# richardshuai/ExPecto

Hardware: AMD Instinct MI355X
Metric: variants/sec (200 windows × 2002 feats) at 1/2/4/8 MI355X; HBM GB/s vs peak (higher is better)
Workload: dtype fp32 in/out (f16x3: power-of-2-scaled 2-way fp16 split = 22-bit operands, 3 MFMA products, fp32 accumulate; bf16x6 recompute on fp16 overflow)

## Files before the change

### expecto_amd/csrc/beluga.hip

```cpp
#include <hip/hip_runtime.h>

#include <algorithm>
#include <array>
#include <cassert>
#include <cstdint>
#include <cstdlib>
#include <cstring>
#include <map>
#include <mutex>
#include <tuple>
#include <string>
#include <vector>

#include "common.h"
#include "gemm_kernel.h"
#include "seg_plan.h"

namespace expecto {

static_assert(kStrandFwd == EXPECTO_STRAND_FWD && kStrandRc == EXPECTO_STRAND_RC && kStrandBoth == EXPECTO_STRAND_BOTH &&
              EXPECTO_EINVAL == -1, "seg_plan.h restates the strand modes and the refusal code");
constexpr int kNFeat = 2002;
constexpr int kFc1In = 67840;
constexpr int kFc1Out = 2003;
// ... 1302 lines not shown
  float* h1 = nullptr;
  long long* a_rows = nullptr;
  long long* c_rows = nullptr;
  int fc2_rows = 0;
  int* win_seg_d = nullptr;
  int* alt_w_d = nullptr;
  int* copy_w_d = nullptr;
  int* seg_var_d = nullptr;
  int seg_var_cap = 0;
  int* win_off_d = nullptr;
  int* win_row_d = nullptr;
  int* fc_perm_d = nullptr;
  hipStream_t st2 = nullptr;
  hipEvent_t pev[16] = {};
  bool overlap = true;
  float* DA = nullptr;
  float* D0 = nullptr;
  float* D1 = nullptr;
  uint8_t* delta_codes = nullptr;
  int* seg_tab = nullptr;
  float* slab_mask = nullptr;
  int win_cap = 0;
  size_t bytes = 0;
  std::vector<void*> allocs;
  int precision = EXPECTO_PRECISION_BF16X6;
  int fc_splits = kFcSplitsDefault;
  int fc2_splits = kFc2SplitsDefault;
  double fc1_m_order_mb = 80.0;
  int fc1_order = 3;
  int fc1_m_group = 8;
  bool fc_wide = true;
  int conv_tile = 0;
  bool conv_ea = true;
  bool fc_skinny = true;
  int fc1_narrow = -1;
  int conv_narrow = -1;
  bool narrow_scope = false;
  int seg_chunk_windows = 0;
  bool seg_merge_strands = true;
  int cus = 0;
  bool pool_one_pass = true;
  bool pool_fused = true;
  float* seam = nullptr;
  float* edge = nullptr;
  size_t seam_cap = 0, edge_cap = 0;
  bool fuse_conv1 = true;
  bool kmer_on = true;
  float* kmer = nullptr;
  uint64_t kmer_key = 0;
  bool kmer_quad = true;
  int kmer_state = 1;
  bool fk_on = true;
  int fk_role = 4;
  float* fkw = nullptr;
  int* fk_sw = nullptr;
  float* fk_cs = nullptr;
  float* fk_seq[3] = {};
  long long fk_seq_rows = 0;
  long long* fk_grows = nullptr;
  long long* fk_wrows = nullptr;
  int* fk_prow = nullptr;
  unsigned* fk_mask = nullptr;
  int fk_slice = 24576;
  float* fk_part = nullptr;
  float* fk_h1 = nullptr;
  long long* fk_arows = nullptr;
// ... 246 lines not shown
    if (idx < 0) return;
    (void)hipEventRecord(h->ev_pool[idx + 1], st);
    h->pending_launch.push_back(rec);
  }
};

struct LayerTimer {
  expecto_beluga* h;
  int layer;
  int idx = -1;
  hipStream_t st;
  LayerTimer(expecto_beluga* hh, int l, hipStream_t s) : h(hh), layer(hh->timer_base + l), st(s) {
    if (!h->profiling) return;
    if (h->ev_next + 2 > h->ev_pool.size()) resolve_events(h);
    idx = (int)h->ev_next;
    h->ev_next += 2;
    (void)hipEventRecord(h->ev_pool[idx], st);
  }
  ~LayerTimer() {
    if (idx < 0) return;
    (void)hipEventRecord(h->ev_pool[idx + 1], st);
    h->pending.push_back({layer, idx});
  }
};

struct DeltaScope {
  expecto_beluga* h;
  explicit DeltaScope(expecto_beluga* hh) : h(hh) { h->timer_base = kNumLayers; }
  ~DeltaScope() { h->timer_base = 0; }
};

thread_local int g_precision = EXPECTO_PRECISION_BF16X6;
thread_local bool g_conv_ea = true;

int act_fmt() {
  return g_precision == EXPECTO_PRECISION_BF16X6 ? 1 : g_precision == EXPECTO_PRECISION_F16X3 ? 2 : 0;
}
int act_bytes() { return act_fmt() == 1 ? 6 : 4; }
bool planes_gemm() { return g_precision != EXPECTO_PRECISION_FP32; }
long long gemm_bm() { return planes_gemm() ? X6P_BM : GBM; }
float exp2i(int e) { return std::ldexp(1.0f, e); }

int conv_tile_rows(const expecto_beluga* h, int l, bool pool, long long M, int n_tiles) {
  if (g_precision != EXPECTO_PRECISION_F16X3) return (int)gemm_bm();
  if (h->conv_tile) return h->conv_tile;
  const int cus = h->cus > 0 ? h->cus : 256;
  auto cost = [&](int bm, double per_row) {
    const long long blocks = (M + bm - 1) / bm * n_tiles;
    return (double)((blocks + cus - 1) / cus) * bm * per_row;
  };
  return cost(384, 1.0) * 1.1 <= cost(256, 1.0) ? 384 : 256;
}

int conv_narrow_cols(int l) { return l == 1 || l == 2 ? 128 : 64; }
bool conv_narrow(const expecto_beluga* h, int l, long long M, int bm, int n_tiles) {
  if (g_precision != EXPECTO_PRECISION_F16X3 || l < 1 || l > 4) return false;
  if (h->conv_narrow >= 0) return h->conv_narrow != 0;
  if (!h->narrow_scope) return false;
  const long long cus = h->cus > 0 ? h->cus : 256;
  const int nc = conv_narrow_cols(l);
  const long long narrow = (M + 255) / 256 * ((kConv[l].cout + nc - 1) / nc), wide = (M + bm - 1) / bm * n_tiles;
  return narrow <= cus && wide < cus;
}

template <int LAYER, int EPI>
int launch_gemm(const GemmArgs& a, int splits, hipStream_t st, int bm = 0) {
// ... 21 lines not shown
          if (g_conv_ea)
            beluga_conv_h3p<LAYER, EPI, 256 | 64 | H3P_FUSE_CONV1, 4><<<dim3((unsigned)nblk), dim3(512), 0, st>>>(a);
          else
            beluga_conv_h3p<LAYER, EPI, 256 | H3P_FUSE_CONV1, 4><<<dim3((unsigned)nblk), dim3(512), 0, st>>>(a);
        } else {
          EXPECTO_REQUIRE(false, "fused conv1: conv2 + pool1 only");
        }
      } else if (a.n_tile_cols == 64) {
        if constexpr ((LAYER == 5 || LAYER == 6) && EPI == EPI_RELU) {
          EXPECTO_REQUIRE(bm == 256 && a.n_tiles * 64 >= a.n_store, "64-column conv tiles: 256 rows");
          beluga_conv_h3p_narrow<LAYER, EPI, 4><<<dim3((unsigned)nblk), dim3(512), 0, st>>>(a);
        } else {
          EXPECTO_REQUIRE(false, "64-column conv tiles: conv5 / conv6 only");
        }
      } else if (a.n_tile_cols == 128) {
        if constexpr (LAYER == 3 || LAYER == 4) {
          EXPECTO_REQUIRE(bm == 256 && a.n_tiles == 4 && a.n_store == 480, "128-column conv tiles: conv3 / conv4");
          beluga_conv_h3p_narrow<LAYER, EPI, 8><<<dim3((unsigned)nblk), dim3(512), 0, st>>>(a);
        } else {
          EXPECTO_REQUIRE(false, "128-column conv tiles: conv3 / conv4 only");
        }
      } else if (bm == 384)
        beluga_conv_h3r<LAYER, EPI><<<dim3((unsigned)nblk), dim3(256), 0, st>>>(a);
      else if (g_conv_ea)
        beluga_conv_h3p<LAYER, EPI, 256 | 64, 4><<<dim3((unsigned)nblk), dim3(512), 0, st>>>(a);
      else
        beluga_conv_h3p<LAYER, EPI, 256, 4><<<dim3((unsigned)nblk), dim3(512), 0, st>>>(a);
    } else if constexpr (EPI == EPI_PARTIAL) {
      EXPECTO_REQUIRE(a.n_tile_cols == 0 || a.n_tile_cols == FCW_BN || a.n_tile_cols == 112 ||
                          a.n_tile_cols == 16 * FCS_NB,
                      "FC tile width: 0 (160), 336, 112 or 32 columns");
      EXPECTO_REQUIRE((long long)a.n_tiles * (a.n_tile_cols ? a.n_tile_cols : GBN) >= a.n_store,
                      "FC N tiles do not cover the stored columns");
      if (a.n_tile_cols == FCW_BN)
        beluga_fc_h3w<LAYER, EPI><<<dim3((unsigned)nblk), dim3(512), 0, st>>>(a);
      else if (a.n_tile_cols == 112)
        beluga_fc_h3w_narrow<LAYER, EPI><<<dim3((unsigned)nblk), dim3(512), 0, st>>>(a);
      else if (a.n_tile_cols == 16 * FCS_NB) {
        EXPECTO_REQUIRE(a.m_tiles == 1 && a.M <= 32 && !a.ks_mask, "skinny FC tiles: one tile of <= 32 rows");
        beluga_fc_h3s<LAYER, EPI><<<dim3((unsigned)nblk), dim3(64 * 2 * FCS_NB), 0, st>>>(a);
      }
      else
        beluga_fc_h3p<LAYER, EPI><<<dim3((unsigned)nblk), dim3(512), 0, st>>>(a);
    } else {
      beluga_fc_h3p<LAYER, EPI><<<dim3((unsigned)nblk), dim3(512), 0, st>>>(a);
    }
  } else
    beluga_gemm<LAYER, EPI, kWM, kMinBlocks, GBK, kPipe><<<dim3((unsigned)nblk), dim3(64 * kWM), 0, st>>>(a);
  return check_launch("beluga_gemm");
}

int run_conv1(expecto_beluga* h, const float* x, const uint8_t* codes, long long code_stride, int n_src, int mode,
              long long row0, int nb, int len, int out_rows, hipStream_t st, float* dst = nullptr) {
  LayerTimer lt(h, 0, st);
  if (h->profiling) h->macs[h->timer_base + 0] += (double)nb * (len - 7) * 320 * 32;
  if (g_precision == EXPECTO_PRECISION_F16X3 && h->w1h) {
    dim3 grid((len - 7 + C1H_ROWS - 1) / C1H_ROWS, nb);
    beluga_conv1_h3<<<grid, dim3(320), 0, st>>>(x, codes, code_stride, n_src, mode, row0,
                                                reinterpret_cast<const _Float16*>(h->w1h), h->cs1, h->b1,
                                                dst ? dst : h->P, out_rows, len, exp2i(h->sx[0]), h->ovf);
    return check_launch("beluga_conv1_h3");
  }
  dim3 grid((len - 7 + C1_T - 1) / C1_T, nb);
  beluga_conv1<<<grid, dim3(320), 0, st>>>(x, codes, code_stride, n_src, mode, row0, h->w1, h->b1,
                                           dst ? dst : h->P, out_rows, len, act_fmt(), exp2i(h->sx[0]), h->ovf);
  return check_launch("beluga_conv1");
}

// ... 451 lines not shown
            g * kFkKb + s * kFkKb / kFkSlabs, kFkKb / kFkSlabs, pr.cnt[g], lay);
      else {
        row += lay;
        ++mslot;
      }
    }
  }
  add(x, w_rows, 100LL * 640, 9 * kFkKb, kFkTailK / GBK, n, n);
  EXPECTO_REQUIRE(G.n <= FCK_MAX && blk < (1LL << 31), "Karatsuba FC1 descriptors");
  EXPECTO_REQUIRE(row <= part_cap, "Karatsuba FC1 partial rows");
  {
    LayerTimer lt(h, 6, st);
    if (h->profiling) {
      if (!mask) {
        h->macs[h->timer_base + 6] += macs;
      } else {
        for (int i = 0; i < G.n; ++i) {
          const FcDesc& d = G.d[i];
          int rc = count_desc_macs(h, d.mask, d.m_tiles, (double)d.M / d.m_tiles * kFc1Out * d.nk * GBK, st);
          if (rc) return rc;
        }
      }
    }
    G.rr = mask ? 0 : 1;
    const long long mtt = blk / G.n_tiles;
    const bool narrow = !mask && fc1_narrow(h, mtt);
    if (narrow) {
      G.n_tiles = kHidLd / (16 * kFcNarrowNb);
      for (int i = 0; i < G.n; ++i) G.d[i].blk0 = G.d[i].blk0 / (kHidLd / FCW_BN) * G.n_tiles;
    }
    const long long grid = G.rr ? (mtt + 7) / 8 * 8 * G.n_tiles : mtt * G.n_tiles;
    if (narrow)
      beluga_fc_h3k_narrow<<<dim3((unsigned)grid), dim3(512), 0, st>>>(G);
    else
      beluga_fc_h3k<0><<<dim3((unsigned)grid), dim3(512), 0, st>>>(G);
    int rc = check_launch("beluga_fc_h3k");
    if (rc) return rc;
  }
  return prow ? fk_reduce(h, part, prow, n, h1, st) : EXPECTO_OK;
}

void fk_slice_tables(const std::vector<FkWin>& ws, int i0, int i1, int T6, std::vector<long long>& grows,
                     FkProducts& pr, std::vector<int>& prow, std::vector<int>* rgrp = nullptr,
                     std::vector<int>* ginfo = nullptr) {
  const int n = i1 - i0;
  std::vector<int> gi(n);
  std::vector<long long> gst;
  std::vector<unsigned> need;
  for (int i = i0; i < i1; ++i) {
    const FkWin& w = ws[i];
    if (i == i0 || !fk_same_group(w, ws[i - 1])) {
      gst.push_back(((long long)w.blk * T6 + fk_group_of(w.off6)) * 640);
      need.push_back(0u);
    }
    gi[i - i0] = (int)gst.size() - 1;
    for (int j = 0; j < 4; ++j) need.back() |= 1u << kFkRole[fk_role_of(w.off6)][j];
    if (ginfo && gi[i - i0] * 2 == (int)ginfo->size()) {
      ginfo->push_back(w.blk);
      ginfo->push_back(fk_group_of(w.off6));
    }
  }
  const int ng = (int)gst.size();
  std::vector<int> ridx((size_t)9 * ng, -1);
  grows.clear();
  if (rgrp) rgrp->clear();
  for (int g = 0; g < 9; ++g) {
    pr.off[g] = (int)grows.size();
    int c = 0;
// ... 36 lines not shown
  return run_fc2(h, h->h1, R, y, st, c_rows);
}

int count_slab_macs(expecto_beluga* h, const unsigned* mask, int tiles, long long nb, hipStream_t st) {
  if (!h->macs_d) {
    float* f = nullptr;
    int rc = dalloc(h, &f, 4 * kNumLayers);
    if (rc) return rc;
    h->macs_d = reinterpret_cast<double*>(f);
    EXPECTO_HIP_CHECK(hipMemsetAsync(h->macs_d, 0, 2 * kNumLayers * sizeof(double), st));
  }
  const double per_bit = (double)nb * kFc1Out * kFc1In / ((double)tiles * h->fc_splits);
  slab_macs<<<dim3(1), dim3(64), 0, st>>>(mask, tiles, per_bit, h->macs_d + kNumLayers + 6);
  return check_launch("slab_macs");
}

int count_desc_macs(expecto_beluga* h, const unsigned* mask, int tiles, double per_tile, hipStream_t st) {
  if (!h->macs_d) {
    float* f = nullptr;
    int rc = dalloc(h, &f, 4 * kNumLayers);
    if (rc) return rc;
    h->macs_d = reinterpret_cast<double*>(f);
    EXPECTO_HIP_CHECK(hipMemsetAsync(h->macs_d, 0, 2 * kNumLayers * sizeof(double), st));
  }
  slab_macs<<<dim3(1), dim3(64), 0, st>>>(mask, tiles, per_tile, h->macs_d + h->timer_base + 6);
  return check_launch("slab_macs");
}

int forward_chunk(expecto_beluga* h, const float* x, const uint8_t* codes, long long code_stride, int n_src,
                  int mode, long long row0, int nb, float* y, hipStream_t st) {
  int rc;
  g_precision = h->precision;
  g_conv_ea = h->conv_ea;
  struct Scope {
    expecto_beluga* h;
    ~Scope() { h->narrow_scope = false; }
  } scope{h};
  h->narrow_scope = true;
  const bool kmer = use_kmer(h, x);
  const bool fuse = !kmer && fuse_conv1(h, x);
  const C1Src f1{codes, code_stride, n_src, mode, row0, kLen};
  if (!kmer && !fuse && (rc = run_conv1(h, x, codes, code_stride, n_src, mode, row0, nb, kLen, kS1, st))) return rc;
  float* src = h->P;
  float* dst = h->Q;
  for (int l = 0; l < 5; ++l) {
    const ConvGeo& g = kConv[l];
    if (l == 0 && kmer)
      rc = run_conv2_kmer(h, f1, nb, g.t_valid, g.s_out, dst, st);
    else
      rc = run_conv(h, l, src, dst, nb, g.s_in, g.t_valid, g.s_out, g.pool != 0, st, l == 0 && fuse ? &f1 : nullptr);
    if (rc) return rc;
    std::swap(src, dst);
  }
  if (fk_use(h)) return fk_windows(h, src, nb, y, st, nullptr);
  return run_fc(h, src, nullptr, nb, y, st);
}

int ensure_delta(expecto_beluga* h) {
  if (h->DA) return EXPECTO_OK;
  const size_t pad = 16 * 640;
  const size_t da = (size_t)h->max_batch * kDA[6] * 640 + pad, dd = (size_t)h->max_batch * kDW[6] * 640 + pad;
  float *pc = nullptr, *tb = nullptr;
  int rc;
  if ((rc = dalloc(h, &h->DA, act_alloc(da))) || (rc = dalloc(h, &h->D0, act_alloc(dd))) ||
      (rc = dalloc(h, &h->D1, act_alloc(dd))) || (rc = dalloc(h, &pc, (size_t)h->max_batch * kC1PatStride / 4)) ||
      (rc = dalloc(h, &tb, (size_t)h->max_batch * kSegTab)) ||
// ... 351 lines not shown
    if (planes_gemm()) {
      const int tiles = (int)((na + gemm_bm() - 1) / gemm_bm());
      unsigned* md = reinterpret_cast<unsigned*>(h->slab_mask);
      EXPECTO_HIP_CHECK(hipMemsetAsync(md, 0, tiles * sizeof(unsigned), st));
      fc1_slab_mask_seg<<<dim3((na + 255) / 256), dim3(256), 0, st>>>(
          widx + f0, na, h->win_seg_d, h->win_off_d, ck.s0, pl.ss, pl.g.L, c.phi, h->seg_tab, (int)gemm_bm(),
          kFc1In / h->fc_splits, md);
      if ((rc = check_launch("fc1_slab_mask_seg"))) return rc;
      mask = md;
      if (h->profiling) {
        if ((rc = count_slab_macs(h, md, tiles, na, st))) return rc;
        frac = 0.0;
      }
    }
    DeltaScope ds(h);
    if (gather2) {
      float* h1a = h1_rows(h, h->fc2_rows);
      if ((rc = run_fc1(h, h->Q, h->a_rows, na, h1a, st, mask, frac, fn)) ||
          (rc = run_fc2(h, h1a, na, pr->y_alt, st, acrow)))
        return rc;
    } else if ((rc = run_fc(h, h->Q, h->a_rows, na, pr->y_alt, st, h->c_rows, mask, frac, fn))) {
      return rc;
    }
  }
  if ((rc = flush2())) return rc;
  return seg_copy_tail(c, ck);
}

int forward_segments(expecto_beluga* h, const uint8_t* codes, int n_seg, int L, long long code_stride, int mode,
                     const int* win_seg, const int* win_off, const int* win_row, int n_win, float* y,
                     hipStream_t st, const SegPairs* pr = nullptr) {
  g_precision = h->precision;
  g_conv_ea = h->conv_ea;
  SegPlan pl;
  const char* refusal = nullptr;
  if (seg_plan({n_seg, L, mode, win_seg, win_off, win_row, n_win, pr ? pr->var_pos : nullptr,
                pr ? pr->strand_stride : n_win, h->max_batch, p_floats(h->max_batch) - 16 * 640,
                q_floats(h->max_batch) - 16 * 640, h->seg_merge_strands, h->seg_chunk_windows, fk_use_seg(h), fk_cap(h)},
               pl, &refusal)) {
    set_error(refusal);
    return EXPECTO_EINVAL;
  }
  int rc;
  if (pr && (rc = ensure_delta(h))) return rc;
  if (n_win > h->win_cap) {
    for (int** b : {&h->win_seg_d, &h->win_off_d, &h->win_row_d, &h->alt_w_d, &h->copy_w_d, &h->fc_perm_d}) {
      if (*b) EXPECTO_HIP_CHECK(hipFree(*b));
      *b = nullptr;
    }
    h->win_cap = 0;
    for (int** b : {&h->win_seg_d, &h->win_off_d, &h->win_row_d}) EXPECTO_HIP_CHECK(hipMalloc(b, n_win * sizeof(int)));
    for (int** b : {&h->alt_w_d, &h->copy_w_d}) EXPECTO_HIP_CHECK(hipMalloc(b, 2 * n_win * sizeof(int)));
    EXPECTO_HIP_CHECK(hipMalloc(&h->fc_perm_d, 4 * n_win * sizeof(int)));
    h->win_cap = n_win;
  }
  if (pr && n_seg > h->seg_var_cap) {
    if (h->seg_var_d) EXPECTO_HIP_CHECK(hipFree(h->seg_var_d));
    h->seg_var_d = nullptr;
    h->seg_var_cap = 0;
    EXPECTO_HIP_CHECK(hipMalloc(&h->seg_var_d, n_seg * sizeof(int)));
    h->seg_var_cap = n_seg;
  }
  std::vector<HostCopy> copies;
  if (pr) {
    copies.push_back({h->seg_var_d, pr->var_pos, n_seg * sizeof(int)});
    copies.push_back({h->alt_w_d, pl.alt_w.data(), pl.alt_w.size() * sizeof(int)});
    copies.push_back({h->copy_w_d, pl.copy_w.data(), pl.copy_w.size() * sizeof(int)});
  }
  if (win_row) copies.push_back({h->win_row_d, win_row, n_win * sizeof(int)});
  copies.push_back({h->win_seg_d, win_seg, n_win * sizeof(int)});
  copies.push_back({h->win_off_d, win_off, n_win * sizeof(int)});
  if (!pl.fc_perm.empty()) copies.push_back({h->fc_perm_d, pl.fc_perm.data(), pl.fc_perm.size() * sizeof(int)});
  if ((rc = stage_copies(h, copies, st))) return rc;
  const SegGeo& g = pl.g;
  const SegCall c{h, pl, st, (pr && h->st2) ? h->st2 : st, pr, SegDims{L, g.T1, g.P1, g.T3, g.T4, g.S5, g.T5, g.T6},
                  make_int4(pl.ph[0], pl.ph[1], pl.ph[2], pl.ph[3]),
                  make_int4(pl.ph_idx[0], pl.ph_idx[1], pl.ph_idx[2], pl.ph_idx[3]), act_bytes(), codes, code_stride,
                  mode, y, win_row ? h->win_row_d : nullptr};
  for (size_t ci = 0; ci < pl.chunks.size(); ++ci) {
    const int s0 = pl.chunks[ci].first, s1 = pl.chunks[ci].second;
    const SegChunk ck{ci, s0, s1 - s0, pl.vfirst[s0], pl.vfirst[s1] - pl.vfirst[s0], (long long)(s1 - s0) * pl.n_ph};
    PQSwap pq{h, false};
    if ((rc = seg_trunk(c, ck, pq))) return rc;
    if (ck.nw > 0 && (rc = pl.fkm ? seg_fc_karatsuba(c, ck) : seg_fc_direct(c, ck))) return rc;
    if (pr && (rc = seg_st_wait(c, h->pev[13]))) return rc;
  }
  return EXPECTO_OK;
}
int forward_pairs(expecto_beluga* h, const uint8_t* ref, const uint8_t* alt, int n, long long stride,
                  const int* var_pos, int mode, float* y_ref, float* y_alt, long long strand_stride, hipStream_t st) {
  g_precision = h->precision;
  g_conv_ea = h->conv_ea;
  const int strands = mode == EXPECTO_STRAND_BOTH ? 2 : 1;
  int rc;
  if ((rc = ensure_delta(h))) return rc;
  const int eb = act_bytes();
  const int nv_max = std::max(1, h->max_batch / strands);
  hipStream_t sa = h->st2 ? h->st2 : st;
  for (int v0 = 0; v0 < n; v0 += nv_max) {
    const int nv = std::min(nv_max, n - v0), R = strands * nv;
    if ((rc = stream_order(st, sa, h->pev[0]))) return rc;
    const bool kmer = use_kmer(h, nullptr);
    const bool fuse = !kmer && fuse_conv1(h, nullptr);
    const C1Src f1{ref + (long long)v0 * stride, stride, nv, mode, 0, kLen};
    if (!kmer && !fuse && (rc = run_conv1(h, nullptr, f1.codes, stride, nv, mode, 0, R, kLen, kS1, st))) return rc;
    if (kmer || fuse) {
      delta_codes2<<<dim3((R + 4) / 5), dim3(5 * kC1PatStride), 0, sa>>>(alt, stride, nv, v0, var_pos, h->delta_codes, R);
      if ((rc = check_launch("delta_codes2"))) return rc;
      DeltaScope ds(h);
      if (fuse && (rc = run_conv1(h, nullptr, h->delta_codes, kC1PatStride, R, EXPECTO_STRAND_FWD, 0, R, kC1Pat, kDA[2],
                                  sa, h->DA)))
        return rc;
    } else {
      delta_codes<<<dim3((R + 15) / 16), dim3(256), 0, sa>>>(alt, stride, nv, v0, var_pos, h->delta_codes, R);
      if ((rc = check_launch("delta_codes"))) return rc;
      DeltaScope ds(h);
      if ((rc = run_conv1(h, nullptr, h->delta_codes, 16, R, EXPECTO_STRAND_FWD, 0, R, kDA[1], kDW[1], sa, h->D0)))
        return rc;
    }
    float* src = h->P;
    float* dst = h->Q;
    float* dprev = h->D0;
    float* dnext = h->D1;
    for (int l = 0; l < 5; ++l) {
      const ConvGeo& g = kConv[l];
// ... 292 lines not shown
    h->fc2_splits = v;
  }
  if (const char* e = getenv("EXPECTO_FC1_M_ORDER_MB")) h->fc1_m_order_mb = atof(e);
  if (const char* e = getenv("EXPECTO_FC1_ORDER")) h->fc1_order = atoi(e);
  if (const char* e = getenv("EXPECTO_FC1_M_GROUP")) h->fc1_m_group = std::max(1, atoi(e));
  if (const char* e = getenv("EXPECTO_FC_WIDE")) h->fc_wide = atoi(e) != 0;
  if (const char* e = getenv("EXPECTO_OVERLAP")) h->overlap = atoi(e) != 0;
  if (const char* e = getenv("EXPECTO_POOL_ONE_PASS")) h->pool_one_pass = atoi(e) != 0;
  if (const char* e = getenv("EXPECTO_POOL_FUSED")) h->pool_fused = atoi(e) != 0;
  if (const char* e = getenv("EXPECTO_FUSE_CONV1")) h->fuse_conv1 = atoi(e) != 0;
  if (const char* e = getenv("EXPECTO_CONV2_TABLE")) h->kmer_on = atoi(e) != 0;
  if (const char* e = getenv("EXPECTO_KMER_QUAD")) h->kmer_quad = atoi(e) != 0;
  if (const char* e = getenv("EXPECTO_ONEHOT_CODES")) h->onehot_as_codes = atoi(e) != 0;
  if (const char* e = getenv("EXPECTO_FC1_KARATSUBA")) h->fk_on = atoi(e) != 0;
  if (const char* e = getenv("EXPECTO_FC1K_SLICE")) h->fk_slice = std::max(1, atoi(e));
  if (const char* e = getenv("EXPECTO_FC1_ROLE")) {
    const int v = atoi(e);
    EXPECTO_REQUIRE(v >= 0 && v <= 4, "EXPECTO_FC1_ROLE must be 0..4");
    h->fk_role = v;
  }
  if (const char* e = getenv("EXPECTO_SEG_CHUNK_WINDOWS")) h->seg_chunk_windows = atoi(e);
  if (const char* e = getenv("EXPECTO_SEG_MERGE_STRANDS")) h->seg_merge_strands = atoi(e) != 0;
  if (const char* e = getenv("EXPECTO_CONV_NARROW")) {
    const int v = atoi(e);
    EXPECTO_REQUIRE(v >= -1 && v <= 1, "EXPECTO_CONV_NARROW must be -1 (auto), 0 or 1");
    h->conv_narrow = v;
  }
  if (const char* e = getenv("EXPECTO_FC1_NARROW")) {
    const int v = atoi(e);
    EXPECTO_REQUIRE(v >= -1 && v <= 1, "EXPECTO_FC1_NARROW must be -1 (auto), 0 or 1");
    h->fc1_narrow = v;
  }
  if (const char* e = getenv("EXPECTO_CONV_EA")) h->conv_ea = atoi(e) != 0;
  if (const char* e = getenv("EXPECTO_FC_SKINNY")) h->fc_skinny = atoi(e) != 0;
  if (const char* e = getenv("EXPECTO_CONV_TILE")) {
    const int v = atoi(e);
    EXPECTO_REQUIRE(v == 0 || v == 256 || v == 384, "EXPECTO_CONV_TILE must be 0 (auto), 256 or 384");
    h->conv_tile = v;
  }
  h->fc2_rows = h->fc2_splits == 1 ? 4 * max_batch : max_batch;
  if (const char* e = getenv("EXPECTO_FC2_ROWS"))
    if (h->fc2_splits == 1) h->fc2_rows = std::max(max_batch, atoi(e));
  const size_t partf = (size_t)std::max(h->fc_splits, kFkParts) * max_batch * kHidLd;
  const size_t h1_rows = (size_t)h->fc2_rows + (h->fc2_splits == 1 ? max_batch : 0);
  if ((rc = dalloc(h, &h->P, act_alloc(pf))) || (rc = dalloc(h, &h->Q, act_alloc(qf))) ||
      (rc = dalloc(h, &h->part, partf)) || (rc = dalloc(h, &h->h1, act_alloc(h1_rows * kHidLd))) ||
      (rc = dalloc(h, &h->part2, (size_t)h->fc2_splits * max_batch * kHidLd)))
    return fail(rc);
  {
    float* rows = nullptr;
    if ((rc = dalloc(h, &rows, (size_t)(max_batch + h1_rows) * 2))) return fail(rc);
    h->a_rows = reinterpret_cast<long long*>(rows);
    h->c_rows = h->a_rows + max_batch;
    float* gr = nullptr;
    if ((rc = dalloc(h, &gr, (size_t)kGresPerBatch * max_batch))) return fail(rc);
    h->fk_gres = reinterpret_cast<int*>(gr);
  }
  EXPECTO_HIP_CHECK(hipMemsetAsync(h->P, 0, act_alloc(pf) * sizeof(float), st));
  EXPECTO_HIP_CHECK(hipMemsetAsync(h->Q, 0, act_alloc(qf) * sizeof(float), st));
  if ((rc = f16_prepare(h, st))) return fail(rc);
  if (h->kmer_on && (rc = kmer_acquire(h, params, st))) return fail(rc);
  h->precision = EXPECTO_PRECISION_F16X3;
  EXPECTO_HIP_CHECK(hipStreamSynchronize(st));
  *out = h;
  return EXPECTO_OK;
}
// ... 338 lines not shown
```

### expecto_amd/csrc/gemm_kernel.h

```cpp
#pragma once
#include <hip/hip_runtime.h>

#include <type_traits>

namespace expecto {

typedef float floatx4 __attribute__((ext_vector_type(4)));
typedef float floatx16 __attribute__((ext_vector_type(16)));

constexpr int GBN = 160;
constexpr int GBK = 32;
constexpr int GTN = GBN / 32;

enum { EPI_RELU = 0, EPI_RELU_POOL4 = 1, EPI_SIGMOID = 2, EPI_PARTIAL = 3, EPI_POOL_PH02 = 4 };

struct GemmArgs {
  const float* A;
  long long lda;
  long long M;
  const float* B;
  long long ldb;
  int kper;
  int taps;
  int n_tiles;
// ... 835 lines not shown
  } else {
    gemm_epilogue16<EPI, 2, 10, 4>(p, acc, m0 + wave * 64, n0, ks, lane);
  }
}

template <int LAYER, int EPI, int TM = 0, int NS = 3>
__global__ __launch_bounds__(512, 1) void beluga_fc_h3p(GemmArgs p) {
  __shared__ __attribute__((aligned(1024))) char smem[NS * FCP_STAGE];
  gemm_fc_h3p_body<LAYER, EPI, TM, NS>(p, smem);
}

constexpr int FCW_NB = 21;
constexpr int FCW_BN = 16 * FCW_NB;
constexpr int FCW_APLANE = 256 * 64;
constexpr int FCW_BPLANE = FCW_NB * 1024;
constexpr int FCW_STAGE = 2 * FCW_APLANE + 2 * FCW_BPLANE;
constexpr int FCW_EROW = 176 * 4 + 16;
constexpr int FCW_EWAVE = 16 * FCW_EROW;

template <int N>
__device__ __forceinline__ void wait_vm() {
  if constexpr (N == 2)
    asm volatile("s_waitcnt vmcnt(2)" ::: "memory");
  else if constexpr (N == 4)
    asm volatile("s_waitcnt vmcnt(4)" ::: "memory");
  else if constexpr (N == 5)
    asm volatile("s_waitcnt vmcnt(5)" ::: "memory");
  else if constexpr (N == 10)
    asm volatile("s_waitcnt vmcnt(10)" ::: "memory");
  else
    static_assert(N == 2, "vmcnt value");
}

template <int NB>
struct FcwGeo {
  static constexpr int BPLANE = NB * 1024;
  static constexpr int STAGE = 2 * FCW_APLANE + 2 * BPLANE;
  static constexpr int JB = (2 * NB + 7) / 8;
  static constexpr int NP = 4 + JB;
  static_assert(2 * STAGE >= 8 * FCW_EWAVE, "epilogue staging inside the stage ring");
};

template <int TM, int NB = FCW_NB, int NS = 2>
__device__ __forceinline__ void fc_h3w_tile(const float* A, const long long* a_rows, long long a_off, long long lda_kb,
                                            int kb0a, long long M, const char* Bb, int kb_total, int nk, float* cbase,
                                            long long ldc, int n_store, long long m0, int n0, char* smem) {
  using G = FcwGeo<NB>;
  constexpr int ROW_KB = 128;
  const int tid = threadIdx.x, lane = tid & 63;
  const int wave = __builtin_amdgcn_readfirstlane(tid >> 6);
  auto swz = [](int r) { return (-(r >> 2)) & 3; };
  const char* asrc[4];
  unsigned adst[4];
  unsigned alive = 0;
#pragma unroll
  for (int i = 0; i < 4; ++i) {
    const int P = wave + 8 * i, g = P >> 1, pl = P & 1;
    if (m0 + 16 * g < M) alive |= 1u << i;
    const int r = 16 * g + (lane >> 2);
    long long m = m0 + r;
    if (m > M - 1) m = M - 1;
    const long long kb0 = (a_rows ? (a_rows[m] + a_off) / GBK : m * lda_kb) + kb0a;
    const int c = (lane & 3) ^ swz(r);
    asrc[i] = (const char*)A + kb0 * ROW_KB + pl * 64 + 16 * c;
    adst[i] = (unsigned)(pl * FCW_APLANE + g * 1024);
  }
  static_assert(G::JB <= 6, "B pieces per wave");
  unsigned boff[6], bdst[6];
#pragma unroll
  for (int j = 0; j < G::JB; ++j) {
    const int Q = min(wave + 8 * j, 2 * NB - 1);
    const int pl = Q / NB, r = 16 * (Q % NB) + (lane >> 2);
    const int c = (lane & 3) ^ swz(r);
    boff[j] = (unsigned)((long long)r * kb_total * ROW_KB + pl * 64 + 16 * c);
    bdst[j] = (unsigned)(2 * FCW_APLANE + Q * 1024);
  }
  const __amdgpu_buffer_rsrc_t brsrc = __builtin_amdgcn_make_buffer_rsrc((void*)Bb, (short)0, 0x7fffffff, 0x00020000);
  auto issue_piece = [&](int s, char* base, int k) {
    if constexpr ((TM & 8) != 0) s = 0;
    if (k < 4) {
      if (NB == FCW_NB || ((alive >> k) & 1u))
        glds16(asrc[k] + (long long)((TM & 16) ? 0 : s) * ROW_KB, base + adst[k]);
    } else
      __builtin_amdgcn_raw_ptr_buffer_load_lds(brsrc, (lds_void*)(base + bdst[k - 4]), 16, boff[k - 4],
                                               (unsigned)(((TM & 32) ? 0 : s) * ROW_KB), 0, 0);
  };

  floatx4v acc[2][NB];
#pragma unroll
  for (int mb = 0; mb < 2; ++mb)
#pragma unroll
    for (int nb = 0; nb < NB; ++nb)
#pragma unroll
      for (int r = 0; r < 4; ++r) acc[mb][nb][r] = 0.f;
  const int fr = lane & 15, fq = lane >> 4;
  const int brow = 2 * FCW_APLANE + fr * 64 + 16 * (fq ^ swz(fr));
  const int arow = (wave * 32 + fr) * 64 + 16 * (fq ^ swz(fr));
  auto read_a = [&](const char* base, bf16x8 (&a)[2][3]) {
#pragma unroll
    for (int mb = 0; mb < 2; ++mb) {
      a[mb][0] = *(const bf16x8*)(base + arow + mb * 1024);
      a[mb][1] = *(const bf16x8*)(base + arow + mb * 1024 + FCW_APLANE);
    }
  };
  auto read_b = [&](const char* base, int nb, bf16x8 (&b)[3]) {
    const char* br = base + brow + nb * 1024;
    b[0] = *(const bf16x8*)(br);
    b[1] = *(const bf16x8*)(br + G::BPLANE);
  };
  auto pin = [&](int nv) {
#pragma unroll
    for (int i = 0; i < 6; ++i) {
      __builtin_amdgcn_sched_group_barrier(0x008, 1, 0);
      if (i == 0 && nv) __builtin_amdgcn_sched_group_barrier(0x020, 1, 0);
      if (i < 2) __builtin_amdgcn_sched_group_barrier(0x100, 1, 0);
      __builtin_amdgcn_sched_group_barrier(0x002, 1, 0);
    }
  };
  static_assert(NS == 2 || NS == 3, "FC ring depth");
  static_assert(NS * G::STAGE <= 160 * 1024, "FC ring in LDS");
  static_assert(NS == 2 || NB != FCW_NB, "3-stage ring: narrow tiles (A pieces of dead row groups skipped)");
  constexpr int LOOK = NS - 1;
  const int npw = __builtin_popcount(alive) + G::JB;
  auto stage_end_wait = [&]() {
    if constexpr (NS == 2) {
      asm volatile("s_waitcnt vmcnt(0)" ::: "memory");
    } else {
      static_assert(G::JB == 2, "vmcnt cases");
      switch (npw) {
        case 2: asm volatile("s_waitcnt vmcnt(2)" ::: "memory"); break;
        case 3: asm volatile("s_waitcnt vmcnt(3)" ::: "memory"); break;
        case 4: asm volatile("s_waitcnt vmcnt(4)" ::: "memory"); break;
        case 5: asm volatile("s_waitcnt vmcnt(5)" ::: "memory"); break;
        default: asm volatile("s_waitcnt vmcnt(6)" ::: "memory"); break;
      }
    }
  };
#pragma unroll
  for (int st = 0; st < LOOK; ++st)
#pragma unroll
    for (int k = 0; k < G::NP; ++k) issue_piece(min(st, nk - 1), smem + st * G::STAGE, k);
  stage_end_wait();
  __builtin_amdgcn_s_barrier();
  asm volatile("" ::: "memory");
  bf16x8 as[2][3];
  bf16x8 b0[3], b1[3];
  const bool live = m0 + 32 * wave < M;
  if (live) {
    for (int s = 0; s < nk; ++s) {
      const char* base = smem + (s % NS) * G::STAGE;
      char* nbase = smem + ((s + LOOK) % NS) * G::STAGE;
      const int s_next = min(s + LOOK, nk - 1);
      constexpr bool more = !(TM & 2);
      read_b(base, 0, b0);
      read_a(base, as);
#pragma unroll
      for (int nb = 0; nb < NB; ++nb) {
        const int k = nb * G::NP / NB;
        const bool issue = more && (nb * G::NP % NB) < G::NP;
        if (issue) issue_piece(s_next, nbase, k);
        if (nb + 1 < NB) read_b(base, nb + 1, (nb & 1) ? b0 : b1);
        __builtin_amdgcn_sched_barrier(0);
#pragma unroll
        for (int mb = 0; mb < 2; ++mb) acc[mb][nb] = planes_mfma<2>(acc[mb][nb], as[mb], (nb & 1) ? b1 : b0);
        pin(issue ? 1 : 0);
      }
      stage_end_wait();
      __builtin_amdgcn_s_barrier();
      asm volatile("" ::: "memory");
    }
  } else {
    for (int s = 0; s < nk; ++s) {
      char* nbase = smem + ((s + LOOK) % NS) * G::STAGE;
      const int s_next = min(s + LOOK, nk - 1);
      if constexpr (!(TM & 2)) {
#pragma unroll
        for (int k = 0; k < G::NP; ++k) issue_piece(s_next, nbase, k);
      }
      stage_end_wait();
      __builtin_amdgcn_s_barrier();
      asm volatile("" ::: "memory");
    }
  }
  if constexpr (NS > 2) {
    asm volatile("s_waitcnt vmcnt(0)" ::: "memory");
    __builtin_amdgcn_s_barrier();
    asm volatile("" ::: "memory");
  }
  if (!live) return;
  char* const lds = smem + wave * FCW_EWAVE;
#pragma unroll
  for (int mb = 0; mb < 2; ++mb) {
#pragma unroll
    for (int h = 0; h < (NB > 11 ? 2 : 1); ++h) {
      const int nb0 = h ? 11 : 0, nbn = NB > 11 ? (h == 0 ? 11 : NB - 11) : NB, cols = 16 * nbn;
#pragma unroll
      for (int nb = 0; nb < 11; ++nb) {
        if (nb >= nbn) break;
#pragma unroll
        for (int j = 0; j < 4; ++j)
          *(float*)(lds + (4 * fq + j) * FCW_EROW + (nb * 16 + fr) * 4) = acc[mb][nb0 + nb][j];
      }
      asm volatile("s_waitcnt lgkmcnt(0)" ::: "memory");
      const int chunks = cols / 4;
      for (int i = lane; i < 16 * chunks; i += 64) {
        const int row = i / chunks, ch = i - row * chunks;
        const long long m = m0 + wave * 32 + mb * 16 + row;
        const int n = n0 + nb0 * 16 + 4 * ch;
        if (m < M && n < n_store)
          *(floatx4v*)(cbase + m * ldc + n) = *(const floatx4v*)(lds + row * FCW_EROW + ch * 16);
      }
      asm volatile("s_waitcnt lgkmcnt(0)" ::: "memory");
    }
  }
}

template <int LAYER, int EPI, int TM, int NB = FCW_NB, int NS = 2>
__device__ __forceinline__ void gemm_fc_h3w_body(const GemmArgs& p, char* smem) {
  static_assert(EPI == EPI_PARTIAL, "split-K partial slabs only");
  const unsigned nblk = gridDim.x, bid = blockIdx.x;
  const unsigned xcd = bid & 7u, q = nblk >> 3, rr = nblk & 7u;
  const unsigned lin =
      p.linear_order ? bid : (xcd < rr ? xcd * (q + 1) : rr * (q + 1) + (xcd - rr) * q) + (bid >> 3);
  long long mt;
  int nt, ks;
  if (p.m_fastest == 3) {
    const long long per_ks = p.m_tiles * p.n_tiles;
    ks = (int)(lin / per_ks);
    const long long r = lin - ks * per_ks;
    const long long g = r / ((long long)p.m_group * p.n_tiles);
    const int i = (int)(r - g * p.m_group * p.n_tiles);
    const int gm = (int)min((long long)p.m_group, p.m_tiles - g * p.m_group);
    nt = i / gm;
    mt = g * p.m_group + i % gm;
  } else if (p.m_fastest) {
    mt = lin % p.m_tiles;
    const long long rest = lin / p.m_tiles;
    nt = (int)(rest % p.n_tiles);
    ks = (int)(rest / p.n_tiles);
  } else {
    nt = (int)(lin % (unsigned)p.n_tiles);
    const long long rest = lin / (unsigned)p.n_tiles;
    mt = rest % p.m_tiles;
    ks = (int)(rest / p.m_tiles);
  }
  if (p.ks_mask && !((p.ks_mask[mt] >> ks) & 1u)) return;
  const long long m0 = mt * X6P_BM;
  const int n0 = nt * 16 * NB;
  const int kb_total = (int)(p.ldb / GBK);
  const int gs0 = ks * (p.kper / GBK);
  constexpr int ROW_KB = 128;
  fc_h3w_tile<TM, NB, NS>(p.A, p.a_rows, 0, p.lda / GBK, gs0, p.M, (const char*)p.Bp + ((long long)n0 * kb_total + gs0) * ROW_KB,
                  kb_total, p.kper / GBK, p.C + (long long)ks * p.split_stride, p.ldc, p.n_store, m0, n0, smem);
}

template <int LAYER, int EPI, int TM = 0>
__global__ __launch_bounds__(512, 1) void beluga_fc_h3w(GemmArgs p) {
  __shared__ __attribute__((aligned(1024))) char smem[2 * FCW_STAGE];
  gemm_fc_h3w_body<LAYER, EPI, TM>(p, smem);
}

template <int LAYER, int EPI>
__global__ __launch_bounds__(512, 1) void beluga_fc_h3w_narrow(GemmArgs p) {
  __shared__ __attribute__((aligned(1024))) char smem[3 * FcwGeo<7>::STAGE];
  gemm_fc_h3w_body<LAYER, EPI, 0, 7, 3>(p, smem);
}

template <int NB>
struct FcsGeo {
  static constexpr int APLANE = 32 * 64;
  static constexpr int BPLANE = NB * 1024;
  static constexpr int STAGE = 2 * APLANE + 2 * BPLANE;
  static constexpr int WAVES = 2 * NB;
  static constexpr int PIECES = 4 + 2 * NB;
};
constexpr int FCS_NB = 2;
constexpr int FCS_NS = 9;
template <int N>
__device__ __forceinline__ void wait_vmn() {
  asm volatile("s_waitcnt vmcnt(%0)" ::"n"(N) : "memory");
}
template <int LAYER, int EPI, int NB = FCS_NB, int NS = FCS_NS>
__global__ __launch_bounds__(64 * 2 * NB, 2) void beluga_fc_h3s(GemmArgs p) {
  static_assert(EPI == EPI_PARTIAL, "split-K partial slabs only");
  using G = FcsGeo<NB>;
  static_assert(2 * NS * G::STAGE <= 160 * 1024, "two workgroups per CU");
  __shared__ __attribute__((aligned(1024))) char smem[NS * G::STAGE];
  constexpr int ROW_KB = 128;
  constexpr int LOOK = NS - 1;
  const int nt = (int)(blockIdx.x % (unsigned)p.n_tiles), ks = (int)(blockIdx.x / (unsigned)p.n_tiles);
// ... 96 lines not shown
  int n, kb_total, n_tiles, n_store;
  long long ldc;
  int rr;
};

template <int TM, int NB, int NS = 2>
__device__ __forceinline__ void fc_h3k_body(const FcGroup& g, char* smem) {
  const unsigned nblk = gridDim.x, bid = blockIdx.x;
  int k = 0, mt, nt;
  if (g.rr) {
    const int slot = (int)(bid >> 3);
    const int T = (slot / g.n_tiles) * 8 + (int)(bid & 7u);
    nt = slot % g.n_tiles;
    while (k + 1 < g.n && T >= g.d[k + 1].blk0 / g.n_tiles) ++k;
    mt = T - g.d[k].blk0 / g.n_tiles;
    if (mt >= g.d[k].m_tiles) return;
  } else {
    const unsigned xcd = bid & 7u, q = nblk >> 3, rr = nblk & 7u;
    const int lin = (int)((xcd < rr ? xcd * (q + 1) : rr * (q + 1) + (xcd - rr) * q) + (bid >> 3));
    while (k + 1 < g.n && lin >= g.d[k + 1].blk0) ++k;
    const int r = lin - g.d[k].blk0;
    nt = r % g.n_tiles;
    mt = r / g.n_tiles;
  }
  const FcDesc& d = g.d[k];
  if (d.mask && !(d.mask[mt] & 1u)) return;
  const int n0 = nt * 16 * NB;
  constexpr int ROW_KB = 128;
  fc_h3w_tile<TM, NB, NS>(d.A, d.a_rows, d.a_off, 0, 0, d.M, d.Bp + (long long)n0 * g.kb_total * ROW_KB, g.kb_total,
                          d.nk, d.C, g.ldc, g.n_store, (long long)mt * X6P_BM, n0, smem);
}

template <int TM = 0>
__global__ __launch_bounds__(512, 1) void beluga_fc_h3k(FcGroup g) {
  __shared__ __attribute__((aligned(1024))) char smem[2 * FcwGeo<FCW_NB>::STAGE];
  fc_h3k_body<TM, FCW_NB>(g, smem);
}

__global__ __launch_bounds__(512, 1) void beluga_fc_h3k_narrow(FcGroup g) {
  __shared__ __attribute__((aligned(1024))) char smem[3 * FcwGeo<7>::STAGE];
  fc_h3k_body<0, 7, 3>(g, smem);
}

constexpr int H3C_AROWS = 288;
constexpr int H3C_APLANE = H3C_AROWS * 64;
constexpr int H3C_ASLAB = 2 * H3C_APLANE;
constexpr int H3C_BSTAGE = 2 * X6P_B_PLANE;
template <int NSB>
constexpr int h3c_lds() { return 2 * H3C_ASLAB + NSB * H3C_BSTAGE; }

template <int MB>
struct SlabGeo {
  static constexpr int BM = 64 * MB;
  static constexpr int GROUPS = MB == 4 ? 18 : (BM + 7 + 15) / 16;
  static constexpr int AROWS = 16 * GROUPS;
  static constexpr int APLANE = AROWS * 64;
  static constexpr int ASLAB = 2 * APLANE;
  static constexpr int PIECES = 2 * GROUPS;
  static constexpr int NA = (PIECES + 3) / 4;
  static constexpr int EXTRA = NA - 8;
  static_assert(AROWS >= BM + 7 && NA >= 8 && NA <= 16, "slab geometry");
};
template <int NSB, int MB>
constexpr int h3c_lds_mb() { return 2 * SlabGeo<MB>::ASLAB + NSB * H3C_BSTAGE; }


template <bool BATCH = true, int NB = 10>
// ... 903 lines not shown
```

Baseline: 1495.

## Retile wide FC kernels into 2D wave grid with 64-row by half-width wave tiles

Adds a new wave layout for the wide FC split-K kernels. By default each of the 8 waves now owns a 64-row by ~11-column-block tile (4 row blocks), replacing the old 32-row by full-width tile. Each wave reads fewer B fragments from LDS per MFMA, and the B loads switch to a per-lane voffset plus per-piece soffset. The old layout stays reachable through EXPECTO_FC_WAVE_TILE=0. A 12-wave variant is defined but not launched. The trade-off is higher accumulator register pressure per wave and a different load-issue schedule.

```diff
diff --git a/expecto_amd/csrc/beluga.hip b/expecto_amd/csrc/beluga.hip
--- a/expecto_amd/csrc/beluga.hip
+++ b/expecto_amd/csrc/beluga.hip
@@ -1358,6 +1358,7 @@
   bool fc_wide = true;
   int conv_tile = 0;
   bool conv_ea = true;
+  bool fc_wave_tile = true;
   bool fc_skinny = true;
   int fc1_narrow = -1;
   int conv_narrow = -1;
@@ -1670,6 +1671,7 @@
 
 thread_local int g_precision = EXPECTO_PRECISION_BF16X6;
 thread_local bool g_conv_ea = true;
+thread_local bool g_fc_wave_tile = true;
 
 int act_fmt() {
   return g_precision == EXPECTO_PRECISION_BF16X6 ? 1 : g_precision == EXPECTO_PRECISION_F16X3 ? 2 : 0;
@@ -1757,8 +1759,10 @@
                       "FC tile width: 0 (160), 336, 112 or 32 columns");
       EXPECTO_REQUIRE((long long)a.n_tiles * (a.n_tile_cols ? a.n_tile_cols : GBN) >= a.n_store,
                       "FC N tiles do not cover the stored columns");
-      if (a.n_tile_cols == FCW_BN)
+      if (a.n_tile_cols == FCW_BN && g_fc_wave_tile)
         beluga_fc_h3w<LAYER, EPI><<<dim3((unsigned)nblk), dim3(512), 0, st>>>(a);
+      else if (a.n_tile_cols == FCW_BN)
+        beluga_fc_h3w<LAYER, EPI, FCW_W32><<<dim3((unsigned)nblk), dim3(512), 0, st>>>(a);
       else if (a.n_tile_cols == 112)
         beluga_fc_h3w_narrow<LAYER, EPI><<<dim3((unsigned)nblk), dim3(512), 0, st>>>(a);
       else if (a.n_tile_cols == 16 * FCS_NB) {
@@ -2276,8 +2280,10 @@
     const long long grid = G.rr ? (mtt + 7) / 8 * 8 * G.n_tiles : mtt * G.n_tiles;
     if (narrow)
       beluga_fc_h3k_narrow<<<dim3((unsigned)grid), dim3(512), 0, st>>>(G);
+    else if (h->fc_wave_tile)
+      beluga_fc_h3k<0><<<dim3((unsigned)grid), dim3(512), 0, st>>>(G);
     else
-      beluga_fc_h3k<0><<<dim3((unsigned)grid), dim3(512), 0, st>>>(G);
+      beluga_fc_h3k<FCW_W32><<<dim3((unsigned)grid), dim3(512), 0, st>>>(G);
     int rc = check_launch("beluga_fc_h3k");
     if (rc) return rc;
   }
@@ -2380,6 +2386,7 @@
   int rc;
   g_precision = h->precision;
   g_conv_ea = h->conv_ea;
+  g_fc_wave_tile = h->fc_wave_tile;
   struct Scope {
     expecto_beluga* h;
     ~Scope() { h->narrow_scope = false; }
@@ -2797,6 +2804,7 @@
                      hipStream_t st, const SegPairs* pr = nullptr) {
   g_precision = h->precision;
   g_conv_ea = h->conv_ea;
+  g_fc_wave_tile = h->fc_wave_tile;
   SegPlan pl;
   const char* refusal = nullptr;
   if (seg_plan({n_seg, L, mode, win_seg, win_off, win_row, n_win, pr ? pr->var_pos : nullptr,
@@ -2856,6 +2864,7 @@
                   const int* var_pos, int mode, float* y_ref, float* y_alt, long long strand_stride, hipStream_t st) {
   g_precision = h->precision;
   g_conv_ea = h->conv_ea;
+  g_fc_wave_tile = h->fc_wave_tile;
   const int strands = mode == EXPECTO_STRAND_BOTH ? 2 : 1;
   int rc;
   if ((rc = ensure_delta(h))) return rc;
@@ -3214,6 +3223,7 @@
     h->fc1_narrow = v;
   }
   if (const char* e = getenv("EXPECTO_CONV_EA")) h->conv_ea = atoi(e) != 0;
+  if (const char* e = getenv("EXPECTO_FC_WAVE_TILE")) h->fc_wave_tile = atoi(e) != 0;
   if (const char* e = getenv("EXPECTO_FC_SKINNY")) h->fc_skinny = atoi(e) != 0;
   if (const char* e = getenv("EXPECTO_CONV_TILE")) {
     const int v = atoi(e);
diff --git a/expecto_amd/csrc/gemm_kernel.h b/expecto_amd/csrc/gemm_kernel.h
--- a/expecto_amd/csrc/gemm_kernel.h
+++ b/expecto_amd/csrc/gemm_kernel.h
@@ -891,30 +891,41 @@
     static_assert(N == 2, "vmcnt value");
 }
 
-template <int NB>
+constexpr int FCW_W32 = 1024;
+constexpr int FCW_W12 = 2048;
+constexpr int fcw_layout(int TM, int NB = FCW_NB) {
+  return NB != FCW_NB || (TM & FCW_W32) ? 0 : (TM & FCW_W12) ? 2 : 1;
+}
+constexpr int fcw_threads(int TM) { return fcw_layout(TM) == 2 ? 768 : 512; }
+
+template <int NB, int WL = 0>
 struct FcwGeo {
+  static constexpr int NW = WL == 2 ? 12 : 8;
+  static constexpr int RB = WL ? 4 : 2;
   static constexpr int BPLANE = NB * 1024;
   static constexpr int STAGE = 2 * FCW_APLANE + 2 * BPLANE;
-  static constexpr int JB = (2 * NB + 7) / 8;
-  static constexpr int NP = 4 + JB;
-  static_assert(2 * STAGE >= 8 * FCW_EWAVE, "epilogue staging inside the stage ring");
+  static constexpr int JA = (32 + NW - 1) / NW;
+  static constexpr int JB = (2 * NB + NW - 1) / NW;
+  static constexpr int NP = JA + JB;
+  static_assert(2 * STAGE >= NW * FCW_EWAVE, "epilogue staging inside the stage ring");
 };
 
-template <int TM, int NB = FCW_NB, int NS = 2>
-__device__ __forceinline__ void fc_h3w_tile(const float* A, const long long* a_rows, long long a_off, long long lda_kb,
+template <int TM, int NB, int NS, int WL, int CBN>
+__device__ __forceinline__ void fc_h3w_part(const float* A, const long long* a_rows, long long a_off, long long lda_kb,
                                             int kb0a, long long M, const char* Bb, int kb_total, int nk, float* cbase,
-                                            long long ldc, int n_store, long long m0, int n0, char* smem) {
-  using G = FcwGeo<NB>;
-  constexpr int ROW_KB = 128;
-  const int tid = threadIdx.x, lane = tid & 63;
-  const int wave = __builtin_amdgcn_readfirstlane(tid >> 6);
+                                            long long ldc, int n_store, long long m0, int n0, char* smem, int wave,
+                                            int row0, int cb0) {
+  using G = FcwGeo<NB, WL>;
+  constexpr int ROW_KB = 128, RB = G::RB, JA = G::JA;
+  const int lane = threadIdx.x & 63;
   auto swz = [](int r) { return (-(r >> 2)) & 3; };
+  static_assert(JA <= 4, "A pieces per wave");
   const char* asrc[4];
   unsigned adst[4];
   unsigned alive = 0;
 #pragma unroll
-  for (int i = 0; i < 4; ++i) {
-    const int P = wave + 8 * i, g = P >> 1, pl = P & 1;
+  for (int i = 0; i < JA; ++i) {
+    const int P = G::NW == 8 ? wave + 8 * i : min(wave + G::NW * i, 31), g = P >> 1, pl = P & 1;
     if (m0 + 16 * g < M) alive |= 1u << i;
     const int r = 16 * g + (lane >> 2);
     long long m = m0 + r;
@@ -928,36 +939,43 @@
   unsigned boff[6], bdst[6];
 #pragma unroll
   for (int j = 0; j < G::JB; ++j) {
-    const int Q = min(wave + 8 * j, 2 * NB - 1);
+    const int Q = min(wave + G::NW * j, 2 * NB - 1);
     const int pl = Q / NB, r = 16 * (Q % NB) + (lane >> 2);
     const int c = (lane & 3) ^ swz(r);
-    boff[j] = (unsigned)((long long)r * kb_total * ROW_KB + pl * 64 + 16 * c);
+    if constexpr (WL == 0)
+      boff[j] = (unsigned)((long long)r * kb_total * ROW_KB + pl * 64 + 16 * c);
+    else
+      boff[j] = (unsigned)((long long)(16 * (Q % NB)) * kb_total * ROW_KB + pl * 64);
     bdst[j] = (unsigned)(2 * FCW_APLANE + Q * 1024);
   }
+  const unsigned boff_lane = (unsigned)((long long)(lane >> 2) * kb_total * ROW_KB + 16 * ((lane & 3) ^ swz(lane >> 2)));
   const __amdgpu_buffer_rsrc_t brsrc = __builtin_amdgcn_make_buffer_rsrc((void*)Bb, (short)0, 0x7fffffff, 0x00020000);
   auto issue_piece = [&](int s, char* base, int k) {
     if constexpr ((TM & 8) != 0) s = 0;
-    if (k < 4) {
+    if (k < JA) {
       if (NB == FCW_NB || ((alive >> k) & 1u))
         glds16(asrc[k] + (long long)((TM & 16) ? 0 : s) * ROW_KB, base + adst[k]);
-    } else
-      __builtin_amdgcn_raw_ptr_buffer_load_lds(brsrc, (lds_void*)(base + bdst[k - 4]), 16, boff[k - 4],
+    } else if constexpr (WL == 0)
+      __builtin_amdgcn_raw_ptr_buffer_load_lds(brsrc, (lds_void*)(base + bdst[k - JA]), 16, boff[k - JA],
                                                (unsigned)(((TM & 32) ? 0 : s) * ROW_KB), 0, 0);
-  };
-
-  floatx4v acc[2][NB];
-#pragma unroll
-  for (int mb = 0; mb < 2; ++mb)
-#pragma unroll
-    for (int nb = 0; nb < NB; ++nb)
+    else
+      __builtin_amdgcn_raw_ptr_buffer_load_lds(brsrc, (lds_void*)(base + bdst[k - JA]), 16, boff_lane,
+                                               boff[k - JA] + (unsigned)(((TM & 32) ? 0 : s) * ROW_KB), 0, 0);
+  };
+
+  floatx4v acc[RB][CBN];
+#pragma unroll
+  for (int mb = 0; mb < RB; ++mb)
+#pragma unroll
+    for (int nb = 0; nb < CBN; ++nb)
 #pragma unroll
       for (int r = 0; r < 4; ++r) acc[mb][nb][r] = 0.f;
   const int fr = lane & 15, fq = lane >> 4;
-  const int brow = 2 * FCW_APLANE + fr * 64 + 16 * (fq ^ swz(fr));
-  const int arow = (wave * 32 + fr) * 64 + 16 * (fq ^ swz(fr));
-  auto read_a = [&](const char* base, bf16x8 (&a)[2][3]) {
-#pragma unroll
-    for (int mb = 0; mb < 2; ++mb) {
+  const int brow = 2 * FCW_APLANE + cb0 * 1024 + fr * 64 + 16 * (fq ^ swz(fr));
+  const int arow = (row0 + fr) * 64 + 16 * (fq ^ swz(fr));
+  auto read_a = [&](const char* base, bf16x8 (&a)[RB][3]) {
+#pragma unroll
+    for (int mb = 0; mb < RB; ++mb) {
       a[mb][0] = *(const bf16x8*)(base + arow + mb * 1024);
       a[mb][1] = *(const bf16x8*)(base + arow + mb * 1024 + FCW_APLANE);
     }
@@ -969,7 +987,7 @@
   };
   auto pin = [&](int nv) {
 #pragma unroll
-    for (int i = 0; i < 6; ++i) {
+    for (int i = 0; i < 3 * RB; ++i) {
       __builtin_amdgcn_sched_group_barrier(0x008, 1, 0);
       if (i == 0 && nv) __builtin_amdgcn_sched_group_barrier(0x020, 1, 0);
       if (i < 2) __builtin_amdgcn_sched_group_barrier(0x100, 1, 0);
@@ -1002,9 +1020,10 @@
   stage_end_wait();
   __builtin_amdgcn_s_barrier();
   asm volatile("" ::: "memory");
-  bf16x8 as[2][3];
+  static_assert(G::NP <= CBN, "at most one piece per MFMA unit");
+  bf16x8 as[RB][3];
   bf16x8 b0[3], b1[3];
-  const bool live = m0 + 32 * wave < M;
+  const bool live = m0 + row0 < M;
   if (live) {
     for (int s = 0; s < nk; ++s) {
       const char* base = smem + (s % NS) * G::STAGE;
@@ -1014,14 +1033,14 @@
       read_b(base, 0, b0);
       read_a(base, as);
 #pragma unroll
-      for (int nb = 0; nb < NB; ++nb) {
-        const int k = nb * G::NP / NB;
-        const bool issue = more && (nb * G::NP % NB) < G::NP;
+      for (int nb = 0; nb < CBN; ++nb) {
+        const int k = nb * G::NP / CBN;
+        const bool issue = more && (nb * G::NP % CBN) < G::NP;
         if (issue) issue_piece(s_next, nbase, k);
-        if (nb + 1 < NB) read_b(base, nb + 1, (nb & 1) ? b0 : b1);
+        if (nb + 1 < CBN) read_b(base, nb + 1, (nb & 1) ? b0 : b1);
         __builtin_amdgcn_sched_barrier(0);
 #pragma unroll
-        for (int mb = 0; mb < 2; ++mb) acc[mb][nb] = planes_mfma<2>(acc[mb][nb], as[mb], (nb & 1) ? b1 : b0);
+        for (int mb = 0; mb < RB; ++mb) acc[mb][nb] = planes_mfma<2>(acc[mb][nb], as[mb], (nb & 1) ? b1 : b0);
         pin(issue ? 1 : 0);
       }
       stage_end_wait();
@@ -1049,10 +1068,10 @@
   if (!live) return;
   char* const lds = smem + wave * FCW_EWAVE;
 #pragma unroll
-  for (int mb = 0; mb < 2; ++mb) {
-#pragma unroll
-    for (int h = 0; h < (NB > 11 ? 2 : 1); ++h) {
-      const int nb0 = h ? 11 : 0, nbn = NB > 11 ? (h == 0 ? 11 : NB - 11) : NB, cols = 16 * nbn;
+  for (int mb = 0; mb < RB; ++mb) {
+#pragma unroll
+    for (int h = 0; h < (CBN > 11 ? 2 : 1); ++h) {
+      const int nb0 = h ? 11 : 0, nbn = CBN > 11 ? (h == 0 ? 11 : CBN - 11) : CBN, cols = 16 * nbn;
 #pragma unroll
       for (int nb = 0; nb < 11; ++nb) {
         if (nb >= nbn) break;
@@ -1064,13 +1083,35 @@
       const int chunks = cols / 4;
       for (int i = lane; i < 16 * chunks; i += 64) {
         const int row = i / chunks, ch = i - row * chunks;
-        const long long m = m0 + wave * 32 + mb * 16 + row;
-        const int n = n0 + nb0 * 16 + 4 * ch;
+        const long long m = m0 + row0 + mb * 16 + row;
+        const int n = n0 + (cb0 + nb0) * 16 + 4 * ch;
         if (m < M && n < n_store)
           *(floatx4v*)(cbase + m * ldc + n) = *(const floatx4v*)(lds + row * FCW_EROW + ch * 16);
       }
       asm volatile("s_waitcnt lgkmcnt(0)" ::: "memory");
     }
+  }
+}
+
+template <int TM, int NB = FCW_NB, int NS = 2>
+__device__ __forceinline__ void fc_h3w_tile(const float* A, const long long* a_rows, long long a_off, long long lda_kb,
+                                            int kb0a, long long M, const char* Bb, int kb_total, int nk, float* cbase,
+                                            long long ldc, int n_store, long long m0, int n0, char* smem) {
+  constexpr int WL = fcw_layout(TM, NB);
+  const int wave = __builtin_amdgcn_readfirstlane(threadIdx.x >> 6);
+  if constexpr (WL == 0) {
+    fc_h3w_part<TM, NB, NS, 0, NB>(A, a_rows, a_off, lda_kb, kb0a, M, Bb, kb_total, nk, cbase, ldc, n_store, m0, n0, smem,
+                                   wave, 32 * wave, 0);
+  } else if constexpr (WL == 1) {
+    if (wave < 4)
+      fc_h3w_part<TM, NB, NS, 1, 11>(A, a_rows, a_off, lda_kb, kb0a, M, Bb, kb_total, nk, cbase, ldc, n_store, m0, n0,
+                                     smem, wave, 64 * wave, 0);
+    else
+      fc_h3w_part<TM, NB, NS, 1, 10>(A, a_rows, a_off, lda_kb, kb0a, M, Bb, kb_total, nk, cbase, ldc, n_store, m0, n0,
+                                     smem, wave, 64 * (wave - 4), 11);
+  } else {
+    fc_h3w_part<TM, NB, NS, 2, 7>(A, a_rows, a_off, lda_kb, kb0a, M, Bb, kb_total, nk, cbase, ldc, n_store, m0, n0, smem,
+                                  wave, 64 * (wave & 3), 7 * (wave >> 2));
   }
 }
 
@@ -1114,7 +1155,7 @@
 }
 
 template <int LAYER, int EPI, int TM = 0>
-__global__ __launch_bounds__(512, 1) void beluga_fc_h3w(GemmArgs p) {
+__global__ __launch_bounds__(fcw_threads(TM), 1) void beluga_fc_h3w(GemmArgs p) {
   __shared__ __attribute__((aligned(1024))) char smem[2 * FCW_STAGE];
   gemm_fc_h3w_body<LAYER, EPI, TM>(p, smem);
 }
@@ -1277,7 +1318,7 @@
 }
 
 template <int TM = 0>
-__global__ __launch_bounds__(512, 1) void beluga_fc_h3k(FcGroup g) {
+__global__ __launch_bounds__(fcw_threads(TM), 1) void beluga_fc_h3k(FcGroup g) {
   __shared__ __attribute__((aligned(1024))) char smem[2 * FcwGeo<FCW_NB>::STAGE];
   fc_h3k_body<TM, FCW_NB>(g, smem);
 }
```

Result: no change. 1508 (median of 6 runs) (+0.9%).
